# vitasoftAI/ImageRetrievalResearch

Measured on AMD Instinct MI355X. Metric: images/sec embed + queries/sec top-k@100k-gallery, EffNet-B3a 224^2, higher is better.
Workload: dtype bf16

## Files before the change

imageretrievalresearch_amd/csrc/mbconv_block.hip:

```cpp
#include "ops.h"

namespace mi355 {

typedef __bf16 bf16x8 __attribute__((ext_vector_type(8)));
typedef float f32x4 __attribute__((ext_vector_type(4)));
typedef unsigned u32x4 __attribute__((ext_vector_type(4)));
typedef unsigned u32x2 __attribute__((ext_vector_type(2)));

constexpr int MB_THREADS = 512;
constexpr int MB_WAVES = MB_THREADS / 64;
constexpr int MB_MAX_RD = 192;
constexpr int MB_MC = MB_WAVES * 16;

__device__ __forceinline__ float mb_lo(unsigned u) { return __uint_as_float(u << 16); }
__device__ __forceinline__ float mb_hi(unsigned u) { return __uint_as_float(u & 0xffff0000u); }

__device__ __forceinline__ void mb_lds_barrier() {
    asm volatile("s_waitcnt lgkmcnt(0)" ::: "memory");
    __builtin_amdgcn_s_barrier();
    asm volatile("" ::: "memory");
}

__host__ __device__ static inline int mb_proj_ntw(int NTp, int MTp, int NTW) {
    int best = 1, best_busy = 0;
// ... 13 lines not shown
    if (wi != 14) return ntw;
    const int nwn = (NTp + ntw - 1) / ntw;
    int msplit = nwn <= MB_WAVES ? MB_WAVES / nwn : 1;
    if (msplit > MTp) msplit = MTp;
    if (nwn <= MB_WAVES && (MTp + msplit - 1) / msplit <= mwp) return ntw;
    return 4;
}

template <int KS> struct MbTaps {
    static constexpr int KK = KS * KS;
    static constexpr int NV = (KS / 2) * KS;
    static constexpr int NH = (KS + 1) / 2;
    static constexpr int NP = NV + NH;
    __host__ __device__ static constexpr bool vertical(int tp) { return tp < NV; }
    __host__ __device__ static constexpr int tap_a(int tp) {
        return tp < NV ? (tp / KS) * 2 * KS + tp % KS : (KS - 1) * KS + (tp - NV) * 2;
    }
    __host__ __device__ static constexpr int tap_b(int tp) {
        return tp < NV ? tap_a(tp) + KS : ((tp - NV) * 2 + 1 < KS ? tap_a(tp) + 1 : -1);
    }
};

template <int KS, int S, int WI, int MW, int MH, int NTW, int MWP, int KST, int A_IT, int ACT_E, int ACT_D>
__global__ __launch_bounds__(MB_THREADS) void k_mbconv_block(const BlockArgs a) {
    using TP = MbTaps<KS>;
    constexpr int MC = MB_MC;
    constexpr int PAD = KS / 2;
    constexpr int NP = TP::NP;
    constexpr int EW = WI + 2 * PAD;
    constexpr int WO = (WI + 2 * PAD - KS) / S + 1;
    constexpr int TR = WO <= 8 ? 2 : 1;
    constexpr int RP = (TR == 2 && S == 1) ? ((EW + 7) & ~7) : EW;
    static_assert(WO <= 16, "depthwise tile geometry");
    constexpr bool PROJ_WHOLE = WI == 7 && NTW == 2;
    constexpr int KC = WI == 7 ? 256 : 128;
    constexpr int ALD = KC + 16;
    extern __shared__ __attribute__((aligned(16))) unsigned char mb_smem[];

    const int tid = threadIdx.x, lane = tid & 63;
    const int wave = __builtin_amdgcn_readfirstlane(tid >> 6);
    const int fr = lane & 15, fq = lane >> 4, fk = fq * 8;
    const int b = blockIdx.x;
    const int P = a.H * a.W, MT = (P + 15) >> 4, XLD = a.XLD;
    const int EH = a.H + 2 * PAD;
    const int EP = (EH + (TR == 2 ? S : 0)) * RP + 8;
    const int Pout = a.Ho * a.Wo;
    const int MTo = TR == 2 ? (a.Ho + 1) >> 1 : a.Ho;
    const int midp = (a.mid + 15) & ~15;

    bf16_t* Xs = reinterpret_cast<bf16_t*>(mb_smem);
    size_t off = ((size_t)MT * 16 * XLD * 2 + 64 + 15) & ~(size_t)15;
    float* pool = reinterpret_cast<float*>(mb_smem + off);
    off += (size_t)((a.mid + 255) & ~255) * 4;
    float* rvec = reinterpret_cast<float*>(mb_smem + off);
    off += MB_MAX_RD * 4;
    unsigned char* R = mb_smem + off;
    bf16_t* Es = reinterpret_cast<bf16_t*>(R) + (size_t)wave * EP * 16;

    const bool stamping = a.stamps != nullptr;
    unsigned t_acc[8] = {0, 0, 0, 0, 0, 0, 0, 0};
    unsigned t_last = 0;
    if (stamping) t_last = (unsigned)__builtin_readcyclecounter();
    auto tick = [&](int i) {
        if (stamping) { const unsigned t = (unsigned)__builtin_readcyclecounter(); t_acc[i] += t - t_last; t_last = t; }
    };
// ... 10 lines not shown
        for (int h = 0; h < KST; ++h) wq[h] = *reinterpret_cast<const u32x4*>(a.We + (n * a.Kp + fk + h * 32));
        be_reg = *reinterpret_cast<const f32x4*>(a.be + min(cbase + wave * 16 + fq * 4, midp - 4));
        __builtin_amdgcn_sched_barrier(0);
    };
    unsigned short wd_raw[NP], wd_nxt[NP];
    f32x4 bd_reg, bd_nxt;
    auto wd_fetch = [&](int cbase) {
        const int ch = min(cbase + wave * 16 + fr, a.mid - 1);
#pragma unroll
        for (int tp = 0; tp < NP; ++tp) {
            const int ta = TP::tap_a(tp), tb = TP::tap_b(tp) < 0 ? TP::tap_a(tp) : TP::tap_b(tp);
            const int t = (lane & 32) ? tb : ta;
            wd_nxt[tp] = a.Wd[t * a.mid + ch];
        }
        bd_nxt = *reinterpret_cast<const f32x4*>(a.bd + min(cbase + wave * 16 + fq * 4, a.mid - 4));
        __builtin_amdgcn_sched_barrier(0);
    };

    w_prefetch_slab(slab_of(0) * MC);
    wd_fetch(slab_of(0) * MC);
    {
        const int kc = (a.Cin + 7) >> 3;
        const int kcl = XLD >> 3;
        const bf16_t* xb = a.X + (size_t)b * P * a.Cin;
        const int total = MT * 16 * kcl;
        constexpr int U = 9;
        for (int id0 = tid; id0 < total; id0 += MB_THREADS * U) {
            u32x4 v[U];
            int dst[U];
#pragma unroll
            for (int u = 0; u < U; ++u) {
                const int id = id0 + u * MB_THREADS;
                const int row = id / kcl, c = id - row * kcl;
                const u32x4 t = *reinterpret_cast<const u32x4*>(xb + (min(row, P - 1) * a.Cin + min(c, kc - 1) * 8));
                const bool ok = id < total && row < P && c < kc;
                v[u] = ok ? t : (u32x4){0u, 0u, 0u, 0u};
                dst[u] = id < total ? row * XLD + c * 8 : -1;
            }
            if (id0 == tid) {
                bf16_t* Eall = reinterpret_cast<bf16_t*>(R);
                for (int id = tid; id < MB_WAVES * EP * 2; id += MB_THREADS)
                    *reinterpret_cast<u32x4*>(&Eall[id * 8]) = (u32x4){0u, 0u, 0u, 0u};
                if (tid < 4) *reinterpret_cast<u32x4*>(&Xs[MT * 16 * XLD + tid * 8]) = (u32x4){0u, 0u, 0u, 0u};
            }
#pragma unroll
            for (int u = 0; u < U; ++u)
                if (dst[u] >= 0) *reinterpret_cast<u32x4*>(&Xs[dst[u]]) = v[u];
        }
    }
    mb_lds_barrier();
    tick(0);

    bf16_t* Db = a.D + (size_t)b * Pout * a.mid;

    const int e_cv = (fq & 1) * 8 + ((fq >> 1) ? RP * 16 : 0);
    const int e_ch = (fq & 1) * 8 + ((fq >> 1) ? 16 : 0);
    const int t_row = TR == 2 ? (fr >> 3) : 0, t_col = TR == 2 ? (fr & 7) : fr;
    const int e_lane = (t_row * S * RP + t_col * S) * 16;
    constexpr int E_TILE = TR * S * RP * 16;
    const bool col_ok = t_col < WO;

    const int abl = a.variant;
    bool prev_active = false;
    for (int ci = 0; ci < nslabs; ++ci) {
        const int cbase = slab_of(ci) * MC;
        const int ch0 = cbase + wave * 16;
        const bool active = ch0 < a.mid;
        {
            constexpr int MTO_SQ = TR == 2 ? (WO + 1) / 2 : WO;
            if (ci > 0 && prev_active && MTo == MTO_SQ) {
                if constexpr (MTO_SQ >= 14) asm volatile("s_waitcnt vmcnt(14)" ::: "memory");
                else if constexpr (MTO_SQ >= 4) asm volatile("s_waitcnt vmcnt(4)" ::: "memory");
                else asm volatile("s_waitcnt vmcnt(1)" ::: "memory");
            } else {
                asm volatile("s_waitcnt vmcnt(0)" ::: "memory");
            }
// ... 436 lines not shown
                        for (int i = 0; i < MWP; ++i) paf[0][i] = *reinterpret_cast<const bf16x8*>(&as[prow[i] + kk * 32]);
                    }
                    __builtin_amdgcn_sched_barrier(0);
                    if (wactive && ch * KPC + kk < KST2) {
    #pragma unroll
                        for (int i = 0; i < MWP; ++i)
    #pragma unroll
                            for (int j = 0; j < NTW; ++j)
                                acc[j][i] = __builtin_amdgcn_mfma_f32_16x16x32_bf16(*reinterpret_cast<bf16x8*>(&cq[kk][j]), paf[AHEAD ? (kk & 1) : 0][i], acc[j][i], 0, 0, 0);
                    }
                    if ((kk & 1) == 1 && ch + 1 < nchunks) {
                        __builtin_amdgcn_sched_barrier(0);
                        c_fetch(ch + 1, kk - 1);
                        c_fetch(ch + 1, kk);
                        __builtin_amdgcn_sched_barrier(0);
                    }
                }
                tick(6);
                mb_lds_barrier();
                tick(6);
            }
        }
        if (wactive) {
            bf16_t* Yb = a.Y + (size_t)b * Pout * a.Cout;
            const bf16_t* Xb = a.X + (size_t)b * P * a.Cin;
            u32x2 rr[NTW][MWP];
            if (a.has_res) {
#pragma unroll
                for (int i = 0; i < MWP; ++i)
#pragma unroll
                    for (int j = 0; j < NTW; ++j) {
                        const int m = min((mt0 + i) * 16 + fr, Pout - 1);
                        const int n = min((wn * ntw + j) * 16 + fq * 4, a.res_n - 4);
                        rr[j][i] = *reinterpret_cast<const u32x2*>(Xb + (m * a.Cin + n));
                    }
                __builtin_amdgcn_sched_barrier(0);
            }
#pragma unroll
            for (int i = 0; i < MWP; ++i) {
                const int m = (mt0 + i) * 16 + fr;
                if (i < mper && m < Pout) {
#pragma unroll
                    for (int j = 0; j < NTW; ++j) {
                        const int n = (wn * ntw + j) * 16 + fq * 4;
                        if (j < ntw && n < a.Cout) {
                            float v[4] = {acc[j][i].x, acc[j][i].y, acc[j][i].z, acc[j][i].w};
                            if (a.has_res && n < a.res_n) {
                                v[0] += mb_lo(rr[j][i].x); v[1] += mb_hi(rr[j][i].x); v[2] += mb_lo(rr[j][i].y); v[3] += mb_hi(rr[j][i].y);
                            }
                            u32x2 o;
                            o.x = pack2bf(v[0], v[1]);
                            o.y = pack2bf(v[2], v[3]);
                            *reinterpret_cast<u32x2*>(Yb + (m * a.Cout + n)) = o;
                        }
                    }
                }
            }
        }
    }
    tick(7);
    if (stamping && tid == 0) {
        long long* o = a.stamps + (size_t)b * 16;
#pragma unroll
        for (int i = 0; i < 8; ++i) o[i] = (long long)t_acc[i];
    }
}

struct MbGeom { int wi, mw, mh, ntw, mwp, a_it; };
static bool mb_geom(int H, int W, MbGeom* g) {
    if (W == 7 && H * W <= 64) { *g = {7, 4, 1, 3, 4, 4}; return true; }
    if (W == 14 && H * W <= 208) { *g = {14, 7, 2, 3, 7, 7}; return true; }
    return false;
}
#define MB_INSTANCES(X)                                                                                              \
    X(3, 1, 14, 3, 3, ACT_SILU) X(5, 1, 14, 3, 3, ACT_SILU) X(5, 1, 14, 5, 3, ACT_SILU) X(5, 2, 14, 5, 2, ACT_SILU)     \
    X(5, 1, 7, 8, 2, ACT_SILU) X(3, 1, 7, 8, 3, ACT_SILU) X(3, 1, 7, 12, 3, ACT_SILU)                                 \
    X(3, 1, 14, 4, 2, ACT_NONE) X(3, 1, 14, 4, 3, ACT_NONE) X(3, 1, 14, 5, 3, ACT_NONE) X(3, 1, 14, 6, 3, ACT_NONE)   \
    X(3, 1, 7, 7, 2, ACT_NONE) X(3, 1, 7, 8, 2, ACT_NONE) X(3, 1, 7, 8, 3, ACT_NONE) X(3, 1, 7, 9, 3, ACT_NONE)       \
    X(3, 1, 7, 10, 3, ACT_NONE) X(3, 1, 7, 11, 3, ACT_NONE) X(3, 1, 14, 6, 4, ACT_NONE)
static bool mb_instance_ok(int k, int stride, int wi, int kst, int ntw, int act_d) {
#define X(KS, S, WI, KST, NTW, AD) if (k == KS && stride == S && wi == WI && kst == KST && ntw == NTW && act_d == AD) return true;
    MB_INSTANCES(X)
#undef X
    return false;
}

static int mb_pick_kcs(const BlockArgs& a) {
    const int Pout = a.Ho * a.Wo;
    const int q = a.W == 7 ? 256 : 128;
    const size_t pl = (size_t)((a.mid + 255) & ~255) * 4;
    const long avail = 160l * 1024 - (long)pl;
    const int kmax = (int)((avail / Pout / 2 - 16) / q) * q;
    if (kmax < q) return 0;
    const int nsc = (a.Kp2 + kmax - 1) / kmax;
    const int per = (a.Kp2 + nsc - 1) / nsc;
    return (per + q - 1) / q * q;
}

static size_t mb_lds_bytes_xld(const BlockArgs& a, int k, int xld, const MbGeom& g) {
    const int P = a.H * a.W, MT = (P + 15) / 16, pad = k / 2;
    const int wo = a.Wo, ew = a.W + 2 * pad;
    const int stride = (a.H + 2 * pad - k) / (a.Ho > 1 ? a.Ho - 1 : 1) >= 2 ? 2 : 1;
    const int rp = (wo <= 8 && stride == 1) ? ((ew + 7) & ~7) : ew;
    const int EP = (a.H + 2 * pad + (wo <= 8 ? stride : 0)) * rp + 8;
    const size_t xs = ((size_t)MT * 16 * xld * 2 + 64 + 15) & ~(size_t)15, pl = (size_t)((a.mid + 255) & ~255) * 4;
    const size_t fixed = xs + pl + MB_MAX_RD * 4;
    const size_t slab = (size_t)MB_WAVES * EP * 16 * 2;
// ... 28 lines not shown
    if (act_e != ACT_SILU) return false;
    if (Cin % 8 || mid % 8 || mid > 2560 || Cout % 8 || rd < 1 || rd > MB_MAX_RD) return false;
    if (!((k == 3 || k == 5) && (stride == 1 || stride == 2))) return false;
    if (W == 7 && stride == 2) return false;
    if ((long)mid * ((Cin + 31) & ~31) >= (1l << 30) || (long)Cout * mid >= (1l << 30)) return false;
    BlockArgs a{};
    a.H = H; a.W = W; a.Cin = Cin; a.Kp = (Cin + 31) & ~31; a.mid = mid; a.Cout = Cout;
    const int pad = k / 2;
    a.Ho = (H + 2 * pad - k) / stride + 1; a.Wo = (W + 2 * pad - k) / stride + 1;
    const int Pout = a.Ho * a.Wo, MTp = (Pout + 15) / 16, NTp = (Cout + 15) / 16;
    const int ntw = mb_pick_ntw(NTp, MTp, g.wi, g.mwp);
    const int nwn = (NTp + ntw - 1) / ntw;
    if (nwn > MB_WAVES) return false;
    int msplit = MB_WAVES / nwn;
    if (msplit > MTp) msplit = MTp;
    if ((MTp + msplit - 1) / msplit > g.mwp) return false;
    a.Kp2 = (mid + 31) & ~31;
    if (Pout * (g.wi == 7 ? 32 : 16) > g.a_it * MB_THREADS) return false;
    if ((H * W + 15) / 16 > g.mw * g.mh) return false;
    if (!mb_instance_ok(k, stride, g.wi, a.Kp / 32, ntw, act_d)) return false;
    return mb_pick_xld(a, k, g) != 0;
}

template <int KS, int S, int WI, int MW, int MH, int NTW, int MWP, int KST, int A_IT, int ACT_E, int ACT_D>
static int launch_mb(BlockArgs a, int B, hipStream_t st) {
    MbGeom g;
    mb_geom(a.H, a.W, &g);
    a.XLD = mb_pick_xld(a, KS, g);
    a.KCS = mb_pick_kcs(a);
    const size_t lds = mb_lds_bytes_xld(a, KS, a.XLD, g);
    static bool attr_done[64] = {false};
    int dev = 0;
    MI355_CHECK_HIP(hipGetDevice(&dev));
    if (dev >= 0 && dev < 64 && !attr_done[dev]) {
        MI355_CHECK_HIP(hipFuncSetAttribute((const void*)k_mbconv_block<KS, S, WI, MW, MH, NTW, MWP, KST, A_IT, ACT_E, ACT_D>,
                                            hipFuncAttributeMaxDynamicSharedMemorySize, 160 * 1024));
        attr_done[dev] = true;
    }
    hipLaunchKernelGGL((k_mbconv_block<KS, S, WI, MW, MH, NTW, MWP, KST, A_IT, ACT_E, ACT_D>), dim3(B), dim3(MB_THREADS), lds, st, a);
    MI355_LAUNCH_CHECK();
    return OK;
}

int launch_mbconv_block(const BlockArgs& a, int B, int k, int stride, hipStream_t st) {
    MI355_REQUIRE(mbconv_block_supported(a.H, a.W, a.Cin, a.mid, a.Cout, k, stride, a.rd, a.act_e, a.act_d), "mbconv_block: unsupported shape");
    const int Pout = a.Ho * a.Wo;
    MbGeom gg;
    mb_geom(a.H, a.W, &gg);
    const int ntw = mb_pick_ntw((a.Cout + 15) / 16, (Pout + 15) / 16, gg.wi, gg.mwp);
    const int kst = a.Kp / 32;
#define X(KS, S, WI, KST, NTW, AD)                                                                  \
    if (k == KS && stride == S && a.W == WI && kst == KST && ntw == NTW && a.act_d == AD)           \
        return launch_mb<KS, S, WI, (WI == 7 ? 4 : 7), (WI == 7 ? 1 : 2), NTW, (WI == 7 ? 4 : 7), KST, (WI == 7 ? 4 : 7), ACT_SILU, AD>(a, B, st);
    MB_INSTANCES(X)
#undef X
    set_error("mbconv_block: no instance for k=%d s=%d W=%d Kp=%d ntw=%d", k, stride, a.W, a.Kp, ntw);
    return ERR_UNSUPPORTED;
}

}
```

imageretrievalresearch_amd/csrc/model.hip:

```cpp
#include "model_exec.h"
#include "../../include/mi355_retrieval.h"

#include <string.h>

#include <algorithm>

namespace mi355 {

int pack_gemm(Packer& pk, Op& op) {
    const TensorSpec* w = pk.get(op.w_name);
    if (!w) return ERR_STATE;
    const int N = op.cout_real, K = op.cin_real;
    MI355_REQUIRE(w->numel() == (int64_t)N * K, "pack: %s has %lld elements, expected %d x %d", op.w_name.c_str(),
                  (long long)w->numel(), N, K);
    std::vector<float> scale, shift;
    if (!pk.bn_fold(op.bn_name, op.bn_eps, N, scale, shift)) return ERR_STATE;
    if (!op.bias_name.empty()) {
        const TensorSpec* b = pk.get(op.bias_name);
        if (!b) return ERR_STATE;
        for (int i = 0; i < N; ++i) shift[i] = b->data[i] * scale[i] + shift[i];
    }
    const int Np = (op.cout + 15) & ~15, Kp = (op.cin + 31) & ~31;
    op.w_off = pk.alloc((size_t)Np * Kp * 2);
    op.b_off = pk.alloc((size_t)Np * 4);
// ... 318 lines not shown
    if (g.out != SLOT_E || d.in != SLOT_E || d.out != SLOT_D || p.in != SLOT_D || !p.use_gate || !d.pool) return false;
    if (g.use_gate || g.res != SLOT_NONE || g.a_relu6 || !g.tap.empty() || !d.tap.empty()) return false;
    if (p.act != ACT_NONE || (p.res != SLOT_NONE && p.res != g.in)) return false;
    if (p.res != SLOT_NONE && p.res_channels && ((p.res_channels + 7) & ~7) != g.cin) return false;
    return mbconv_block_supported(h, w, g.cin, g.cout, p.cout, d.k, d.stride, s.rd, g.act, d.act);
}

static int stamp_ptr(ExecCtx& cx, size_t oi, long long** out) {
    mi355_model* m = cx.m;
    *out = nullptr;
    if (!m->block_stamps) return OK;
    const size_t need = m->def.ops.size() * (size_t)cx.B * 16 * sizeof(long long);
    if (m->stamp_bytes < need) {
        if (m->stamp_buf) MI355_CHECK_HIP(hipFree(m->stamp_buf));
        MI355_CHECK_HIP(hipMalloc((void**)&m->stamp_buf, need));
        m->stamp_bytes = need;
    }
    m->stamp_B = cx.B;
    *out = m->stamp_buf + (oi * (size_t)cx.B + cx.b0) * 16;
    MI355_CHECK_HIP(hipMemsetAsync(*out, 0, (size_t)cx.nb * 16 * sizeof(long long), cx.st));
    return OK;
}

static int exec_block(ExecCtx& cx, size_t oi) {
    mi355_model* m = cx.m;
    SlotState* S = m->slots;
    const Op& g = m->def.ops[oi];
    const Op& d = m->def.ops[oi + 1];
    const Op& s = m->def.ops[oi + 2];
    const Op& p = m->def.ops[oi + 3];
    BlockArgs a{};
    a.X = (const bf16_t*)cx.slot_ptr(g.in);
    a.We = (const bf16_t*)cx.w(g.w_off); a.be = (const float*)cx.w(g.b_off);
    a.Wd = (const bf16_t*)cx.w(d.w_off); a.bd = (const float*)cx.w(d.b_off);
    a.W1 = (const bf16_t*)cx.w(s.w3_off); a.b1 = (const float*)cx.w(s.b_off);
    a.W2 = (const bf16_t*)cx.w(s.w4_off); a.b2 = (const float*)cx.w(s.b2_off);
    a.Wp = (const bf16_t*)cx.w(p.w_off); a.bp = (const float*)cx.w(p.b_off);
    a.D = (bf16_t*)cx.slot_ptr(d.out);
    a.Y = (bf16_t*)cx.slot_ptr(p.out);
    a.H = S[g.in].h; a.W = S[g.in].w; a.Cin = g.cin; a.Kp = (g.cin + 31) & ~31; a.mid = g.cout;
    a.Ho = S[d.out].h; a.Wo = S[d.out].w; a.Cout = p.cout; a.Kp2 = (p.cin + 31) & ~31; a.rd = s.rd;
    a.has_res = p.res != SLOT_NONE;
    a.res_n = p.res != SLOT_NONE ? (p.res_channels ? ((p.res_channels + 7) & ~7) : p.cout) : 0;
    a.a_relu6 = p.a_relu6;
    a.act_e = g.act; a.act_d = d.act; a.se_act = s.se_act;
    a.inv_hw = 1.0f / (float)(a.Ho * a.Wo);
    a.norot = m->block_norot;
    a.variant = m->block_variant;
    a.stamps = nullptr;
    { const int rc = stamp_ptr(cx, oi, &a.stamps); if (rc != OK) return rc; }
    return launch_mbconv_block(a, cx.nb, d.k, d.stride, cx.st);
}

static int exec_fused(ExecCtx& cx, const Op& g, const Op& d) {
    mi355_model* m = cx.m;
    SlotState* S = m->slots;
    FusedArgs a{};
    a.X = (const bf16_t*)cx.slot_ptr(g.in);
    a.We = (const bf16_t*)cx.w(g.w_off); a.be = (const float*)cx.w(g.b_off);
    a.Wd = (const bf16_t*)cx.w(d.w_off); a.bd = (const float*)cx.w(d.b_off);
    a.D = (bf16_t*)cx.slot_ptr(d.out);
    a.pool = d.pool ? (float*)cx.slot_ptr(SLOT_POOLPART) : nullptr;
    a.H = S[g.in].h; a.W = S[g.in].w; a.Cin = g.cin; a.Kp = (g.cin + 31) & ~31; a.mid = g.cout;
    a.Ho = S[d.out].h; a.Wo = S[d.out].w; a.act_e = g.act; a.act_d = d.act;
    a.debug_skip = m->fuse_debug;
    if (fused_late_supported(a.H, a.W, g.cin, g.cout, d.k, d.stride)) {
        m->pool_nblk = 1;
        return launch_fused_late(a, cx.nb, d.k, d.stride, cx.st);
    }
    if (use_sweep(m, g, d, a.H, a.W)) {
        SweepArgs sa{};
        sa.X = a.X; sa.We = a.We; sa.be = a.be; sa.Wd = a.Wd; sa.bd = a.bd; sa.D = a.D; sa.pool = a.pool;
        sa.H = a.H; sa.W = a.W; sa.Cin = a.Cin; sa.Kp = a.Kp; sa.mid = a.mid; sa.Ho = a.Ho; sa.Wo = a.Wo;
        sa.act_e = a.act_e; sa.act_d = a.act_d; sa.csplit_override = m->sweep_csplit; sa.variant = m->sweep_variant; sa.debug_skip = m->sweep_skip;
// ... 6 lines not shown
    return launch_fused_band(a, cx.nb, d.k, d.stride, cx.st);
}

static void op_range_label(const Op& op, int H, int W, int in_h, int in_w, const char* how, char* lab, size_t n) {
    switch (op.kind) {
        case OP_STEM: snprintf(lab, n, "embed/%sstem 3->%d @%dx%d", how, op.cout_real, conv_out(H, 3, 2), conv_out(W, 3, 2)); break;
        case OP_GEMM: snprintf(lab, n, "embed/%spw %d->%d @%dx%d%s%s", how, op.cin_real, op.cout_real, in_h, in_w,
                               op.use_gate ? " gate" : "", op.res != SLOT_NONE ? " res" : ""); break;
        case OP_DW: snprintf(lab, n, "embed/%sdw k%d s%d C%d @%dx%d", how, op.k, op.stride, op.cin_real, in_h, in_w); break;
        case OP_SE: snprintf(lab, n, "embed/%sse C%d rd%d", how, op.cin_real, op.rd); break;
        default: snprintf(lab, n, "embed/%sop%d C%d->%d t%d", how, (int)op.kind, op.cin_real, op.cout_real, op.tokens_h); break;
    }
}

static int run_backbone(ExecCtx& cx, size_t op_begin = 0, size_t op_end = (size_t)-1) {
    mi355_model* m = cx.m;
    SlotState* S = m->slots;
    if (op_end > m->def.ops.size()) op_end = m->def.ops.size();
    for (size_t oi = op_begin; oi < op_end; ++oi) {
        const Op& op = m->def.ops[oi];
        const int op_index = (int)oi;
        const int in_h = S[op.in == SLOT_NONE ? 0 : op.in].h, in_w = S[op.in == SLOT_NONE ? 0 : op.in].w;
        const bool block = op.in != SLOT_NONE && can_fuse_block(m, oi, in_h, in_w, cx.B);
        const bool fused = block || can_fuse(m, oi, in_h, in_w);
        if (fused) {
            const Op& d = m->def.ops[oi + 1];
            S[op.out].h = S[op.in].h; S[op.out].w = S[op.in].w; S[op.out].c = op.cout;
            S[d.out].h = conv_out(S[op.in].h, d.k, d.stride); S[d.out].w = conv_out(S[op.in].w, d.k, d.stride);
            S[d.out].c = d.cout;
            if (block) {
                const Op& pj = m->def.ops[oi + 3];
                S[pj.out].h = S[d.out].h; S[pj.out].w = S[d.out].w; S[pj.out].c = pj.cout;
            }
        } else
        switch (op.kind) {
            case OP_STEM: S[op.out].h = conv_out(cx.H, 3, 2); S[op.out].w = conv_out(cx.W, 3, 2); S[op.out].c = op.cout; break;
            case OP_GEMM: S[op.out].h = S[op.in].h; S[op.out].w = S[op.in].w; S[op.out].c = op.cout; break;
            case OP_DW: {
                const int ho = conv_out(S[op.in].h, op.k, op.stride), wo = conv_out(S[op.in].w, op.k, op.stride);
                S[op.out].h = ho; S[op.out].w = wo; S[op.out].c = op.cout;
                break;
            }
            case OP_SE: break;
            default: if (op.out != SLOT_NONE) { S[op.out].h = op.tokens_h; S[op.out].w = op.tokens_h; S[op.out].c = op.cout; } break;
        }
        hipEvent_t e0 = nullptr, e1 = nullptr;
// ... 167 lines not shown
    m->def.num_classes = num_classes;
    const std::string n = name;
    int e;
    if (n == "efficientnet_b3a" || n == "efficientnet_b3") e = build_efficientnet_b3(m->def);
    else if (n == "rexnet_100") e = build_rexnet(m->def, 1.0);
    else if (n == "rexnet_130") e = build_rexnet(m->def, 1.3);
    else if (n == "rexnet_150") e = build_rexnet(m->def, 1.5);
    else if (n == "rexnet_200") e = build_rexnet(m->def, 2.0);
    else if (n == "swin_base_patch4_window7_224") e = build_swin_base(m->def);
    else {
        set_error("Unknown model name '%s'. Known: efficientnet_b3a, rexnet_100/130/150/200, swin_base_patch4_window7_224", name);
        e = ERR_ARG;
    }
    if (e) { delete m; return e; }
    *out = m;
    return OK;
}

void mi355_model_destroy(mi355_model_t m) {
    if (!m) return;
    if (m->dev_blob) (void)hipFree(m->dev_blob);
    if (m->arena) (void)hipFree(m->arena);
    if (m->stamp_buf) (void)hipFree(m->stamp_buf);
    for (int l = 0; l < 4; ++l) {
        if (m->lane_stream[l]) (void)hipStreamDestroy(m->lane_stream[l]);
        if (m->lane_join[l]) (void)hipEventDestroy(m->lane_join[l]);
    }
    if (m->lane_fork) (void)hipEventDestroy(m->lane_fork);
    for (auto& kv : m->tapbufs)
        if (kv.second.ptr) (void)hipFree(kv.second.ptr);
    delete m;
}

int mi355_model_num_tensors(mi355_model_t m) { return m ? (int)m->def.tensors.size() : 0; }

int mi355_model_tensor_info(mi355_model_t m, int i, const char** name, int* ndim, int64_t shape[4], int* kind) {
    MI355_REQUIRE(m && i >= 0 && i < (int)m->def.tensors.size(), "tensor_info: index %d out of range", i);
    const TensorSpec& t = m->def.tensors[i];
    if (name) *name = t.name.c_str();
    if (ndim) *ndim = (int)t.shape.size();
    if (shape)
        for (int d = 0; d < 4; ++d) shape[d] = d < (int)t.shape.size() ? t.shape[d] : 1;
    if (kind) *kind = t.kind;
    return OK;
}

// ... 61 lines not shown
    size_t i0 = ops.size(), i1 = ops.size();
    for (size_t i = 0; i < ops.size(); ++i) {
        if (ops[i].tap == from_tap) i0 = i;
        if (ops[i].tap == to_tap) i1 = i;
    }
    MI355_REQUIRE(i0 < ops.size() && i1 < ops.size() && i0 < i1, "run_between_taps: taps '%s' -> '%s' not found in that order",
                  from_tap, to_tap);
    const Op& src = ops[i0];
    MI355_REQUIRE(src.out != SLOT_NONE && (src.cout_real ? src.cout_real : src.cout) == C,
                  "run_between_taps: tap '%s' has %d channels, got %d", from_tap, src.cout_real ? src.cout_real : src.cout, C);
    hipStream_t st = (hipStream_t)stream;
    int H = 32, W = 32;
    for (const Op& op : ops) { (void)op; }
    {
        int sh = 1;
        for (size_t i = 0; i <= i0; ++i)
            if (ops[i].kind == OP_STEM || (ops[i].kind == OP_DW && ops[i].stride == 2)) sh *= 2;
        H = h * sh; W = w * sh;
    }
    const size_t bytes = plan_slots(m, B, H, W);
    m->lane_bytes = 0;
    if (int e = ensure_arena(m, bytes)) return e;
    ExecCtx cx{m, st, B, H, W, nullptr, 0, B};
    SlotState* S = m->slots;
    S[src.out].h = h; S[src.out].w = w; S[src.out].c = src.cout;
    if (int e = launch_nchw_f32_to_nhwc_bf16(x, (bf16_t*)cx.slot_ptr(src.out), B, h * w, C, src.cout, st)) return e;
    return run_backbone(cx, i0 + 1, i1 + 1);
}

int mi355_model_forward_u8(mi355_model_t m, const unsigned char* images, int B, int h, int w, int fill, const float* mean,
                           const float* stdv, const float* conv_input_w, int features_only, float* out, float* pooled_out,
                           void* stream) {
    MI355_REQUIRE(m && images && mean && stdv && out, "forward_u8: null pointer");
    MI355_REQUIRE(B >= 1 && h >= 1 && w >= 1 && h <= 16384 && w <= 16384, "forward_u8: bad image size %dx%d", h, w);
    MI355_REQUIRE(fill >= 0 && fill <= 255, "forward_u8: fill must be a byte value");
    for (int c = 0; c < 3; ++c) MI355_REQUIRE(stdv[c] != 0.f, "forward_u8: std[%d] is zero", c);
    MI355_REQUIRE(!m->def.ops.empty() && (m->def.ops[0].kind == OP_STEM || m->def.ops[0].kind == OP_PATCH_EMBED),
                  "forward_u8: %s has no stem / patch embedding to fuse the pre-processing into", m->def.arch.c_str());
    MI355_REQUIRE(m->def.ops[0].kind == OP_STEM || !conv_input_w, "forward_u8: conv_input belongs to the convolutional backbones");
    U8Source u{};
    u.img = images; u.h = h; u.w = w; u.fill = fill; u.conv_w = conv_input_w;
    for (int c = 0; c < 3; ++c) { u.mean[c] = mean[c]; u.stdv[c] = stdv[c]; }
    const int S = h > w ? h : w;
    return forward_impl(m, nullptr, B, S, S, out, pooled_out, features_only != 0, (hipStream_t)stream, &u);
}

// ... 61 lines not shown
    MI355_REQUIRE(it != m->tapbufs.end(), "read_tap: no tap named '%s' was recorded", tap_name);
    const TapBuf& t = it->second;
    if (shape) { shape[0] = t.B; shape[1] = t.c_real; shape[2] = t.h; shape[3] = t.w; }
    if (!out) return OK;
    MI355_REQUIRE(out_numel >= (int64_t)t.B * t.c_real * t.h * t.w, "read_tap: output too small");
    return launch_nhwc_to_nchw_f32((const bf16_t*)t.ptr, out, t.B, t.h * t.w, t.c, t.c_real, (hipStream_t)stream);
}

int mi355_model_set_option(mi355_model_t m, const char* key, int64_t value) {
    MI355_REQUIRE(m && key, "set_option: null argument");
    const std::string k = key;
    if (k == "microbatch") m->microbatch = (int)value;
    else if (k == "lanes") m->lanes = (int)value;
    else if (k == "fuse") m->fuse = value != 0;
    else if (k == "fuse_band") m->fuse_band = (int)value;
    else if (k == "fuse_sweep") m->fuse_sweep = (int)value;
    else if (k == "sweep_csplit") m->sweep_csplit = (int)value;
    else if (k == "sweep_variant") m->sweep_variant = (int)value;
    else if (k == "sweep_skip") m->sweep_skip = (int)value;
    else if (k == "fuse_debug") m->fuse_debug = (int)value;
    else if (k == "fuse_ln") m->fuse_ln = (int)value;
    else if (k == "fuse_block") m->fuse_block = (int)value;
    else if (k == "fuse_block_min_batch") m->fuse_block_min_batch = (int)value;
    else if (k == "block_stamps") m->block_stamps = value != 0;
    else if (k == "block_norot") m->block_norot = (int)value;
    else if (k == "block_variant") m->block_variant = (int)value;
    else if (k == "fuse_head_gap") m->fuse_head_gap = value != 0;
    else if (k == "roctx") roctx_enable(value != 0);
    else if (k == "profile") {
        m->profile = value != 0;
        for (int i = 0; i < PK_COUNT; ++i) { m->prof_ms[i] = 0; m->prof_launches[i] = 0; }
        m->prof_op_ms.assign(m->def.ops.size(), 0.0);
        m->prof_op_n.assign(m->def.ops.size(), 0);
    } else {
        set_error("set_option: unknown option '%s'", key);
        return ERR_ARG;
    }
    return OK;
}

int mi355_model_profile_read(mi355_model_t m, double* ms_by_kind, int64_t* launches_by_kind, int n) {
    MI355_REQUIRE(m && ms_by_kind && launches_by_kind && n >= PK_COUNT, "profile_read: need arrays of >= %d", PK_COUNT);
    for (auto& pe : m->prof_events) {
        MI355_CHECK_HIP(hipEventSynchronize(pe.second.second));
        float ms = 0.f;
        MI355_CHECK_HIP(hipEventElapsedTime(&ms, pe.second.first, pe.second.second));
// ... 233 lines not shown
```

imageretrievalresearch_amd/csrc/model_exec.h:

```cpp
#pragma once
#include "model.h"

#include <string.h>

namespace mi355 {

int swin_exec(const ModelDef& def, const Op& op, struct ExecCtx& cx);

static inline uint16_t f2bf_host(float f) {
    uint32_t u;
    memcpy(&u, &f, 4);
    if ((u & 0x7fffffffu) > 0x7f800000u) return (uint16_t)((u >> 16) | 0x40);
    u += 0x7fffu + ((u >> 16) & 1u);
    return (uint16_t)(u >> 16);
}
static inline float bf_round_host(float f) {
    uint32_t u = ((uint32_t)f2bf_host(f)) << 16;
    float r;
    memcpy(&r, &u, 4);
    return r;
}

struct SlotState {
    size_t off = 0, bytes = 0;
// ... 15 lines not shown
struct mi355_model {
    ModelDef def;
    std::vector<char> blob;
    void* dev_blob = nullptr;
    size_t dev_blob_bytes = 0;
    bool packed = false;
    void* arena = nullptr;
    size_t arena_bytes = 0;
    int arena_device = -1, blob_device = -1;
    SlotState slots[SLOT_COUNT];
    int microbatch = 0;
    int lanes = 1;
    hipStream_t lane_stream[4] = {nullptr, nullptr, nullptr, nullptr};
    hipEvent_t lane_fork = nullptr, lane_join[4] = {nullptr, nullptr, nullptr, nullptr};
    size_t lane_bytes = 0;
    int fuse_sweep = 1;
    int sweep_variant = 0, sweep_skip = 0;
    int sweep_csplit = 0;
    int fuse_band = 2;
    bool fuse = true;
    int fuse_block = 1;
    int fuse_block_min_batch = 96;
    bool fuse_head_gap = true;
    int block_variant = 0;
    int block_norot = 0;
    bool block_stamps = false;
    long long* stamp_buf = nullptr; size_t stamp_bytes = 0; int stamp_B = 0;
    int fuse_debug = 0;
    int fuse_ln = 1;
    int pool_nblk = 0;
    bool taps = false;
    std::map<std::string, TapBuf> tapbufs;
    bool profile = false;
    std::vector<std::pair<int, std::pair<hipEvent_t, hipEvent_t>>> prof_events;
    std::vector<char> prof_fused;
    std::vector<double> prof_op_ms;
    std::vector<long> prof_op_n;
    double prof_ms[PK_COUNT] = {0};
    long prof_launches[PK_COUNT] = {0};
};

namespace mi355 {

struct ExecCtx {
    mi355_model* m;
    hipStream_t st;
    int nb, H, W;
    const float* x;
    int b0, B;
    int lane = 0;
    const unsigned char* x_u8 = nullptr;
    int img_h = 0, img_w = 0, fill = 255;
    float mean[3] = {0.f, 0.f, 0.f}, stdv[3] = {1.f, 1.f, 1.f};
    const float* conv_w = nullptr;
    const int64_t* u8_desc = nullptr;
    int ln_pending_in = SLOT_NONE;
    char* base() const { return (char*)m->arena + (size_t)lane * m->lane_bytes; }
    void* slot_ptr(int s) const { return s == SLOT_NONE ? nullptr : base() + m->slots[s].off; }
    const char* w(size_t off) const { return (const char*)m->dev_blob + off; }
};

struct Packer {
    mi355_model* m;
    std::vector<char>& blob;
    size_t alloc(size_t bytes) {
        const size_t off = align_up(blob.size(), 256);
        blob.resize(off + bytes, 0);
        return off;
    }
    const TensorSpec* get(const std::string& name) {
        auto it = m->def.index.find(name);
        if (it == m->def.index.end()) { set_error("pack: unknown tensor '%s'", name.c_str()); return nullptr; }
        const TensorSpec& t = m->def.tensors[it->second];
        if (!t.set) { set_error("pack: tensor '%s' was never set (mi355_model_set_tensor)", name.c_str()); return nullptr; }
        return &t;
    }
    bool bn_fold(const std::string& bn, float eps, int n, std::vector<float>& scale, std::vector<float>& shift) {
        scale.assign(n, 1.f);
        shift.assign(n, 0.f);
// ... 17 lines not shown
```

imageretrievalresearch_amd/csrc/ops.h:

```cpp
#pragma once
#include "common.h"

namespace mi355 {

struct GemmArgs {
    const bf16_t* A; int lda;
    const bf16_t* W; int ldw;
    const float* bias;
    const bf16_t* res; int ldr; int res_n;
    const float* gate; int gate_ld; int rows_per_img;
    void* out; int ldo; int out_f32;
    int M, N, K;
    int act;
    int a_relu6;
    const bf16_t* zeros;
    long M_sel;
    float* splitk_ws;
    size_t splitk_ws_bytes;
    const float* ln_stats;
    const float* ln_colsum;
};
int launch_gemm_bf16(const GemmArgs& a, hipStream_t st, int* path = nullptr);
bool gemm_wide_supported(const GemmArgs& a);
int launch_gemm_wide(const GemmArgs& a, hipStream_t st);
// ... 37 lines not shown
bool sweep_mbconv_supported(int H, int W, int Cin, int mid, int k, int stride, int act_e, int act_d);
int launch_sweep_mbconv(const SweepArgs& a, int B, int k, int stride, hipStream_t st);

struct BlockArgs {
    const bf16_t* X;
    const bf16_t* We; const float* be;
    const bf16_t* Wd; const float* bd;
    const bf16_t* W1; const float* b1;
    const bf16_t* W2; const float* b2;
    const bf16_t* Wp; const float* bp;
    bf16_t* D;
    bf16_t* Y;
    long long* stamps;
    int H, W, Cin, Kp, mid, Ho, Wo, Cout, Kp2, rd;
    int XLD;
    int KCS;
    int norot;
    int variant;
    int has_res;
    int res_n;
    int a_relu6;
    int act_e, act_d, se_act;
    float inv_hw;
};
bool mbconv_block_supported(int H, int W, int Cin, int mid, int Cout, int k, int stride, int rd, int act_e, int act_d);
int launch_mbconv_block(const BlockArgs& a, int B, int k, int stride, hipStream_t st);

int launch_stem(const float* x, const float* w, const float* bias, bf16_t* out, int B, int H, int W, int Cout,
                int act, hipStream_t st);

int launch_stem_u8(const unsigned char* img, int h, int w, int fill, const float* mean, const float* stdv,
                   const float* conv_w, const float* sw, const float* bias, bf16_t* out, int B, int Cout, int act,
                   hipStream_t st, const int64_t* desc = nullptr, int b0 = 0);

int check_images(const unsigned char* pixels, int64_t pixels_bytes, const int64_t* desc_host, const int64_t* desc_dev, int B,
                 const char* who);
size_t resize_batch_workspace(const int64_t* desc_host, int B, int out_h, int out_w, bool pad);
int resize_batch(const unsigned char* pixels, int64_t pixels_bytes, const int64_t* desc_host, const int64_t* desc_dev, int B,
                 int out_h, int out_w, bool pad, int fill, unsigned char* out, void* workspace, size_t workspace_bytes,
                 hipStream_t st);

int dw_pool_blocks(int Ho, int Wo, int C);
int launch_dwconv(const bf16_t* in, const bf16_t* w, const float* bias, bf16_t* out, float* pool_partial, int B,
                  int H, int W, int C, int k, int stride, int act, int* pool_nblk, hipStream_t st);

int launch_se(const float* pool_partial, int nblk, float inv_hw, const float* w1, const float* b1, const float* w2,
              const float* b2, float* gate, int B, int C, int rd, int act1, hipStream_t st);

int launch_gap(const bf16_t* in, float* pooled, bf16_t* pooled_bf16, int B, int HW, int C, hipStream_t st);
// ... 17 lines not shown
```

Measured before the change: 60270.

## Fuse consecutive MBConv blocks into one persistent chain kernel launch

Adds a chain kernel that runs several consecutive fused MBConv blocks inside one launch. Each workgroup handles one image and dispatches per-block template instances through a switch over a device-side entry table. Intermediate outputs ping-pong between two halves of the E slot, with per-entry batch strides. The aim is to remove per-block launch overhead and inter-kernel gaps and to keep each image's data hot in cache. The cost is a much larger combined kernel, which risks register pressure and code bloat and makes occupancy follow the worst block. It also adds host-side table management with an async memcpy when entries change.

New measurement: 60230 (median of 6 runs). Within noise of the previous version (-0.1%).

```diff
diff --git a/imageretrievalresearch_amd/csrc/mbconv_block.hip b/imageretrievalresearch_amd/csrc/mbconv_block.hip
--- a/imageretrievalresearch_amd/csrc/mbconv_block.hip
+++ b/imageretrievalresearch_amd/csrc/mbconv_block.hip
@@ -59,7 +59,7 @@
 };
 
 template <int KS, int S, int WI, int MW, int MH, int NTW, int MWP, int KST, int A_IT, int ACT_E, int ACT_D>
-__global__ __launch_bounds__(MB_THREADS) void k_mbconv_block(const BlockArgs a) {
+__device__ __forceinline__ void mb_block_body(const BlockArgs& a, const int b, const int tid) {
     using TP = MbTaps<KS>;
     constexpr int MC = MB_MC;
     constexpr int PAD = KS / 2;
@@ -74,10 +74,9 @@
     constexpr int ALD = KC + 16;
     extern __shared__ __attribute__((aligned(16))) unsigned char mb_smem[];
 
-    const int tid = threadIdx.x, lane = tid & 63;
+    const int lane = tid & 63;
     const int wave = __builtin_amdgcn_readfirstlane(tid >> 6);
     const int fr = lane & 15, fq = lane >> 4, fk = fq * 8;
-    const int b = blockIdx.x;
     const int P = a.H * a.W, MT = (P + 15) >> 4, XLD = a.XLD;
     const int EH = a.H + 2 * PAD;
     const int EP = (EH + (TR == 2 ? S : 0)) * RP + 8;
@@ -134,7 +133,7 @@
     {
         const int kc = (a.Cin + 7) >> 3;
         const int kcl = XLD >> 3;
-        const bf16_t* xb = a.X + (size_t)b * P * a.Cin;
+        const bf16_t* xb = a.X + (size_t)b * a.xs;
         const int total = MT * 16 * kcl;
         constexpr int U = 9;
         for (int id0 = tid; id0 < total; id0 += MB_THREADS * U) {
@@ -163,7 +162,7 @@
     mb_lds_barrier();
     tick(0);
 
-    bf16_t* Db = a.D + (size_t)b * Pout * a.mid;
+    bf16_t* Db = a.D + (size_t)b * a.ds;
 
     const int e_cv = (fq & 1) * 8 + ((fq >> 1) ? RP * 16 : 0);
     const int e_ch = (fq & 1) * 8 + ((fq >> 1) ? 16 : 0);
@@ -646,8 +645,8 @@
             }
         }
         if (wactive) {
-            bf16_t* Yb = a.Y + (size_t)b * Pout * a.Cout;
-            const bf16_t* Xb = a.X + (size_t)b * P * a.Cin;
+            bf16_t* Yb = a.Y + (size_t)b * a.ys;
+            const bf16_t* Xb = a.X + (size_t)b * a.xs;
             u32x2 rr[NTW][MWP];
             if (a.has_res) {
 #pragma unroll
@@ -690,6 +689,11 @@
     }
 }
 
+template <int KS, int S, int WI, int MW, int MH, int NTW, int MWP, int KST, int A_IT, int ACT_E, int ACT_D>
+__global__ __launch_bounds__(MB_THREADS) void k_mbconv_block(const BlockArgs a) {
+    mb_block_body<KS, S, WI, MW, MH, NTW, MWP, KST, A_IT, ACT_E, ACT_D>(a, blockIdx.x, threadIdx.x);
+}
+
 struct MbGeom { int wi, mw, mh, ntw, mwp, a_it; };
 static bool mb_geom(int H, int W, MbGeom* g) {
     if (W == 7 && H * W <= 64) { *g = {7, 4, 1, 3, 4, 4}; return true; }
@@ -702,11 +706,48 @@
     X(3, 1, 14, 4, 2, ACT_NONE) X(3, 1, 14, 4, 3, ACT_NONE) X(3, 1, 14, 5, 3, ACT_NONE) X(3, 1, 14, 6, 3, ACT_NONE)   \
     X(3, 1, 7, 7, 2, ACT_NONE) X(3, 1, 7, 8, 2, ACT_NONE) X(3, 1, 7, 8, 3, ACT_NONE) X(3, 1, 7, 9, 3, ACT_NONE)       \
     X(3, 1, 7, 10, 3, ACT_NONE) X(3, 1, 7, 11, 3, ACT_NONE) X(3, 1, 14, 6, 4, ACT_NONE)
+#define MB_TARGS(KS, S, WI, KST, NTW, AD) \
+    KS, S, WI, (WI == 7 ? 4 : 7), (WI == 7 ? 1 : 2), NTW, (WI == 7 ? 4 : 7), KST, (WI == 7 ? 4 : 7), ACT_SILU, AD
+struct MbInst { int ks, s, wi, kst, ntw, ad; };
+#define X(KS, S, WI, KST, NTW, AD) MbInst{KS, S, WI, KST, NTW, AD},
+constexpr MbInst MB_TABLE[] = {MB_INSTANCES(X)};
+#undef X
+constexpr int MB_NINST = sizeof(MB_TABLE) / sizeof(MB_TABLE[0]);
+__host__ __device__ constexpr int mb_inst_id(int k, int stride, int wi, int kst, int ntw, int act_d) {
+    for (int i = 0; i < MB_NINST; ++i) {
+        const MbInst& t = MB_TABLE[i];
+        if (t.ks == k && t.s == stride && t.wi == wi && t.kst == kst && t.ntw == ntw && t.ad == act_d) return i;
+    }
+    return -1;
+}
 static bool mb_instance_ok(int k, int stride, int wi, int kst, int ntw, int act_d) {
-#define X(KS, S, WI, KST, NTW, AD) if (k == KS && stride == S && wi == WI && kst == KST && ntw == NTW && act_d == AD) return true;
-    MB_INSTANCES(X)
+    return mb_inst_id(k, stride, wi, kst, ntw, act_d) >= 0;
+}
+
+template <int ACT_D>
+__global__ __launch_bounds__(MB_THREADS) void k_mbconv_chain(const MbChainEntry* ents, int n) {
+#if defined(__HIP_DEVICE_COMPILE__)
+    typedef const __attribute__((address_space(4))) MbChainEntry* CPtr;
+#else
+    typedef const MbChainEntry* CPtr;
+#endif
+    const CPtr ce = (CPtr)ents;
+    for (int i = 0; i < n; ++i) {
+        if (i > 0) __syncthreads();
+        int b = blockIdx.x, tid = threadIdx.x;
+        asm volatile("" : "+s"(b));
+        asm volatile("" : "+v"(tid));
+        const BlockArgs a = ce[i].a;
+        switch (ce[i].inst) {
+#define X(KS, S, WI, KST, NTW, AD) \
+            case mb_inst_id(KS, S, WI, KST, NTW, AD):                                                                 \
+                if constexpr (AD == ACT_D) mb_block_body<MB_TARGS(KS, S, WI, KST, NTW, AD)>(a, b, tid);                 \
+                break;
+            MB_INSTANCES(X)
 #undef X
-    return false;
+            default: break;
+        }
+    }
 }
 
 static int mb_pick_kcs(const BlockArgs& a) {
@@ -781,40 +822,73 @@
     return mb_pick_xld(a, k, g) != 0;
 }
 
-template <int KS, int S, int WI, int MW, int MH, int NTW, int MWP, int KST, int A_IT, int ACT_E, int ACT_D>
-static int launch_mb(BlockArgs a, int B, hipStream_t st) {
+static int mb_prepare(BlockArgs& a, int k, int stride, size_t* lds) {
     MbGeom g;
     mb_geom(a.H, a.W, &g);
-    a.XLD = mb_pick_xld(a, KS, g);
+    a.XLD = mb_pick_xld(a, k, g);
     a.KCS = mb_pick_kcs(a);
-    const size_t lds = mb_lds_bytes_xld(a, KS, a.XLD, g);
-    static bool attr_done[64] = {false};
+    if (!a.xs) a.xs = a.H * a.W * a.Cin;
+    if (!a.ds) a.ds = a.Ho * a.Wo * a.mid;
+    if (!a.ys) a.ys = a.Ho * a.Wo * a.Cout;
+    *lds = mb_lds_bytes_xld(a, k, a.XLD, g);
+    const int Pout = a.Ho * a.Wo;
+    const int ntw = mb_pick_ntw((a.Cout + 15) / 16, (Pout + 15) / 16, g.wi, g.mwp);
+    return mb_inst_id(k, stride, g.wi, a.Kp / 32, ntw, a.act_d);
+}
+
+static int mb_lds_attr(const void* fn, bool (&done)[64]) {
     int dev = 0;
     MI355_CHECK_HIP(hipGetDevice(&dev));
-    if (dev >= 0 && dev < 64 && !attr_done[dev]) {
-        MI355_CHECK_HIP(hipFuncSetAttribute((const void*)k_mbconv_block<KS, S, WI, MW, MH, NTW, MWP, KST, A_IT, ACT_E, ACT_D>,
-                                            hipFuncAttributeMaxDynamicSharedMemorySize, 160 * 1024));
-        attr_done[dev] = true;
-    }
+    if (dev >= 0 && dev < 64 && !done[dev]) {
+        MI355_CHECK_HIP(hipFuncSetAttribute(fn, hipFuncAttributeMaxDynamicSharedMemorySize, 160 * 1024));
+        done[dev] = true;
+    }
+    return OK;
+}
+
+template <int KS, int S, int WI, int MW, int MH, int NTW, int MWP, int KST, int A_IT, int ACT_E, int ACT_D>
+static int launch_mb(const BlockArgs& a, size_t lds, int B, hipStream_t st) {
+    static bool attr_done[64] = {false};
+    if (int e = mb_lds_attr((const void*)k_mbconv_block<KS, S, WI, MW, MH, NTW, MWP, KST, A_IT, ACT_E, ACT_D>, attr_done)) return e;
     hipLaunchKernelGGL((k_mbconv_block<KS, S, WI, MW, MH, NTW, MWP, KST, A_IT, ACT_E, ACT_D>), dim3(B), dim3(MB_THREADS), lds, st, a);
     MI355_LAUNCH_CHECK();
     return OK;
 }
 
-int launch_mbconv_block(const BlockArgs& a, int B, int k, int stride, hipStream_t st) {
-    MI355_REQUIRE(mbconv_block_supported(a.H, a.W, a.Cin, a.mid, a.Cout, k, stride, a.rd, a.act_e, a.act_d), "mbconv_block: unsupported shape");
-    const int Pout = a.Ho * a.Wo;
-    MbGeom gg;
-    mb_geom(a.H, a.W, &gg);
-    const int ntw = mb_pick_ntw((a.Cout + 15) / 16, (Pout + 15) / 16, gg.wi, gg.mwp);
-    const int kst = a.Kp / 32;
-#define X(KS, S, WI, KST, NTW, AD)                                                                  \
-    if (k == KS && stride == S && a.W == WI && kst == KST && ntw == NTW && a.act_d == AD)           \
-        return launch_mb<KS, S, WI, (WI == 7 ? 4 : 7), (WI == 7 ? 1 : 2), NTW, (WI == 7 ? 4 : 7), KST, (WI == 7 ? 4 : 7), ACT_SILU, AD>(a, B, st);
+int launch_mbconv_block(const BlockArgs& a0, int B, int k, int stride, hipStream_t st) {
+    MI355_REQUIRE(mbconv_block_supported(a0.H, a0.W, a0.Cin, a0.mid, a0.Cout, k, stride, a0.rd, a0.act_e, a0.act_d), "mbconv_block: unsupported shape");
+    BlockArgs a = a0;
+    size_t lds = 0;
+    const int id = mb_prepare(a, k, stride, &lds);
+#define X(KS, S, WI, KST, NTW, AD) \
+    if (id == mb_inst_id(KS, S, WI, KST, NTW, AD)) return launch_mb<MB_TARGS(KS, S, WI, KST, NTW, AD)>(a, lds, B, st);
     MB_INSTANCES(X)
 #undef X
-    set_error("mbconv_block: no instance for k=%d s=%d W=%d Kp=%d ntw=%d", k, stride, a.W, a.Kp, ntw);
+    set_error("mbconv_block: no instance for k=%d s=%d W=%d Kp=%d", k, stride, a.W, a.Kp);
     return ERR_UNSUPPORTED;
 }
 
-}
+size_t mbconv_chain_entry(const BlockArgs& a, int k, int stride, MbChainEntry* e) {
+    *e = MbChainEntry{};
+    if (!mbconv_block_supported(a.H, a.W, a.Cin, a.mid, a.Cout, k, stride, a.rd, a.act_e, a.act_d)) return 0;
+    e->a = a;
+    size_t lds = 0;
+    e->inst = mb_prepare(e->a, k, stride, &lds);
+    return e->inst >= 0 ? lds : 0;
+}
+
+int mbconv_chain_family(const MbChainEntry& e) { return e.inst >= 0 && e.inst < MB_NINST ? MB_TABLE[e.inst].ad : -1; }
+
+bool mbconv_chain_family_supported(int family) { return family == ACT_SILU; }
+
+int launch_mbconv_chain(const MbChainEntry* entries, int n, int family, size_t lds, int B, hipStream_t st) {
+    MI355_REQUIRE(entries && n >= 1 && B >= 1 && lds >= 1 && lds <= 160 * 1024, "mbconv_chain: bad arguments");
+    MI355_REQUIRE(mbconv_chain_family_supported(family), "mbconv_chain: no chain kernel for family %d", family);
+    static bool attr_done[64] = {false};
+    if (int e = mb_lds_attr((const void*)k_mbconv_chain<ACT_SILU>, attr_done)) return e;
+    hipLaunchKernelGGL(k_mbconv_chain<ACT_SILU>, dim3(B), dim3(MB_THREADS), lds, st, entries, n);
+    MI355_LAUNCH_CHECK();
+    return OK;
+}
+
+}
diff --git a/imageretrievalresearch_amd/csrc/model.hip b/imageretrievalresearch_amd/csrc/model.hip
--- a/imageretrievalresearch_amd/csrc/model.hip
+++ b/imageretrievalresearch_amd/csrc/model.hip
@@ -364,9 +364,8 @@
     return OK;
 }
 
-static int exec_block(ExecCtx& cx, size_t oi) {
+static BlockArgs block_args(ExecCtx& cx, size_t oi, int h, int w, int ho, int wo) {
     mi355_model* m = cx.m;
-    SlotState* S = m->slots;
     const Op& g = m->def.ops[oi];
     const Op& d = m->def.ops[oi + 1];
     const Op& s = m->def.ops[oi + 2];
@@ -380,8 +379,8 @@
     a.Wp = (const bf16_t*)cx.w(p.w_off); a.bp = (const float*)cx.w(p.b_off);
     a.D = (bf16_t*)cx.slot_ptr(d.out);
     a.Y = (bf16_t*)cx.slot_ptr(p.out);
-    a.H = S[g.in].h; a.W = S[g.in].w; a.Cin = g.cin; a.Kp = (g.cin + 31) & ~31; a.mid = g.cout;
-    a.Ho = S[d.out].h; a.Wo = S[d.out].w; a.Cout = p.cout; a.Kp2 = (p.cin + 31) & ~31; a.rd = s.rd;
+    a.H = h; a.W = w; a.Cin = g.cin; a.Kp = (g.cin + 31) & ~31; a.mid = g.cout;
+    a.Ho = ho; a.Wo = wo; a.Cout = p.cout; a.Kp2 = (p.cin + 31) & ~31; a.rd = s.rd;
     a.has_res = p.res != SLOT_NONE;
     a.res_n = p.res != SLOT_NONE ? (p.res_channels ? ((p.res_channels + 7) & ~7) : p.cout) : 0;
     a.a_relu6 = p.a_relu6;
@@ -390,8 +389,121 @@
     a.norot = m->block_norot;
     a.variant = m->block_variant;
     a.stamps = nullptr;
+    return a;
+}
+
+static int exec_block(ExecCtx& cx, size_t oi) {
+    SlotState* S = cx.m->slots;
+    const Op& g = cx.m->def.ops[oi];
+    const Op& d = cx.m->def.ops[oi + 1];
+    BlockArgs a = block_args(cx, oi, S[g.in].h, S[g.in].w, S[d.out].h, S[d.out].w);
     { const int rc = stamp_ptr(cx, oi, &a.stamps); if (rc != OK) return rc; }
     return launch_mbconv_block(a, cx.nb, d.k, d.stride, cx.st);
+}
+
+static bool read_before_write(const mi355_model* m, size_t from, int slot) {
+    for (size_t i = from; i < m->def.ops.size(); ++i) {
+        const Op& op = m->def.ops[i];
+        if (op.in == slot || op.res == slot || (op.use_gate && slot == SLOT_GATE)) return true;
+        if (op.out == slot) return false;
+    }
+    return false;
+}
+
+static int exec_chain(ExecCtx& cx, size_t oi, size_t op_end, int* launched) {
+    mi355_model* m = cx.m;
+    SlotState* S = m->slots;
+    const auto& ops = m->def.ops;
+    *launched = 0;
+    if (!m->fuse_chain || m->profile || m->block_stamps || m->taps || !cx.chain_ok) return OK;
+    struct Blk { size_t oi; int h, w, ho, wo; };
+    std::vector<Blk> run;
+    {
+        int h = S[ops[oi].in].h, w = S[ops[oi].in].w;
+        for (size_t j = oi; j + 3 < op_end && ops[j].in != SLOT_NONE && can_fuse_block(m, j, h, w, cx.B); j += 4) {
+            if (!run.empty() && ops[j].in != ops[run.back().oi + 3].out) break;
+            const Op& d = ops[j + 1];
+            const Blk bk{j, h, w, conv_out(h, d.k, d.stride), conv_out(w, d.k, d.stride)};
+            run.push_back(bk);
+            h = bk.ho; w = bk.wo;
+        }
+    }
+    std::vector<MbChainEntry> ents;
+    for (size_t n = run.size(); n >= 2; --n) {
+        const Blk& f = run[0];
+        const Blk& l = run[n - 1];
+        const Op& g0 = ops[f.oi];
+        const Op& pl = ops[l.oi + 3];
+        const int s_in = g0.in, s_out = pl.out;
+        if (s_in == SLOT_E || s_in == SLOT_D || s_out == SLOT_E || s_out == SLOT_D) continue;
+        const long x0 = (long)f.h * f.w * g0.cin, yl = (long)l.ho * l.wo * pl.cout;
+        if (s_in == s_out && x0 != yl) continue;
+        long ymax = 0, dmax = 0;
+        for (size_t k = 0; k < n; ++k) {
+            const Blk& bk = run[k];
+            if (k + 1 < n) ymax = std::max(ymax, (long)bk.ho * bk.wo * ops[bk.oi + 3].cout);
+            dmax = std::max(dmax, (long)bk.ho * bk.wo * ops[bk.oi].cout);
+        }
+        const size_t half = (S[SLOT_E].bytes / 2) & ~(size_t)255;
+        if ((size_t)cx.nb * ymax * 2 > half || (size_t)cx.nb * dmax * 2 > S[SLOT_D].bytes) continue;
+        const size_t after = l.oi + 4;
+        bool stale = read_before_write(m, after, SLOT_E) || read_before_write(m, after, SLOT_D);
+        for (size_t k = 0; k + 1 < n && !stale; ++k) {
+            const int so = ops[run[k].oi + 3].out;
+            if (so != s_out && read_before_write(m, after, so)) stale = true;
+        }
+        if (stale) continue;
+        bf16_t* ebuf[2] = {(bf16_t*)cx.slot_ptr(SLOT_E), (bf16_t*)((char*)cx.slot_ptr(SLOT_E) + half)};
+        ents.assign(n, MbChainEntry{});
+        size_t lds = 0;
+        int family = -1;
+        bool ok = true;
+        for (size_t k = 0; k < n && ok; ++k) {
+            const Blk& bk = run[k];
+            BlockArgs a = block_args(cx, bk.oi, bk.h, bk.w, bk.ho, bk.wo);
+            if (k > 0) { a.X = ebuf[(k - 1) & 1]; a.xs = (int)ymax; }
+            if (k + 1 < n) { a.Y = ebuf[k & 1]; a.ys = (int)ymax; }
+            a.ds = (int)dmax;
+            const Op& d = ops[bk.oi + 1];
+            const size_t l_k = mbconv_chain_entry(a, d.k, d.stride, &ents[k]);
+            const int fam = mbconv_chain_family(ents[k]);
+            ok = l_k > 0 && mbconv_chain_family_supported(fam) && (family < 0 || fam == family);
+            family = fam;
+            lds = std::max(lds, l_k);
+        }
+        if (!ok) continue;
+        const size_t nops = ops.size(), base = (size_t)cx.lane * nops + f.oi;
+        int dev = 0;
+        MI355_CHECK_HIP(hipGetDevice(&dev));
+        if (!m->chain_dev || m->chain_device != dev || m->chain_host.size() != 4 * nops) {
+            if (m->chain_dev) (void)hipFree(m->chain_dev);
+            m->chain_dev = nullptr;
+            MI355_CHECK_HIP(hipMalloc((void**)&m->chain_dev, 4 * nops * sizeof(MbChainEntry)));
+            m->chain_device = dev;
+            m->chain_host.assign(4 * nops, MbChainEntry{});
+            for (auto& e : m->chain_host) e.inst = -1;
+        }
+        if (memcmp(&m->chain_host[base], ents.data(), n * sizeof(MbChainEntry)) != 0) {
+            memcpy(&m->chain_host[base], ents.data(), n * sizeof(MbChainEntry));
+            MI355_CHECK_HIP(hipMemcpyAsync(m->chain_dev + base, &m->chain_host[base], n * sizeof(MbChainEntry), hipMemcpyHostToDevice, cx.st));
+        }
+        char lab[96] = "";
+        if (roctx_active()) snprintf(lab, sizeof lab, "embed/block chain: %d blocks from op %d", (int)n, (int)f.oi);
+        RoctxRange range(lab);
+        if (int e = launch_mbconv_chain(m->chain_dev + base, (int)n, family, lds, cx.nb, cx.st)) return e;
+        for (size_t k = 0; k < n; ++k) {
+            const Blk& bk = run[k];
+            const Op& g = ops[bk.oi];
+            const Op& d = ops[bk.oi + 1];
+            const Op& p = ops[bk.oi + 3];
+            S[g.out].h = bk.h; S[g.out].w = bk.w; S[g.out].c = g.cout;
+            S[d.out].h = bk.ho; S[d.out].w = bk.wo; S[d.out].c = d.cout;
+            S[p.out].h = bk.ho; S[p.out].w = bk.wo; S[p.out].c = p.cout;
+        }
+        *launched = (int)n;
+        return OK;
+    }
+    return OK;
 }
 
 static int exec_fused(ExecCtx& cx, const Op& g, const Op& d) {
@@ -444,6 +556,11 @@
         const int op_index = (int)oi;
         const int in_h = S[op.in == SLOT_NONE ? 0 : op.in].h, in_w = S[op.in == SLOT_NONE ? 0 : op.in].w;
         const bool block = op.in != SLOT_NONE && can_fuse_block(m, oi, in_h, in_w, cx.B);
+        if (block) {
+            int n = 0;
+            if (int e = exec_chain(cx, oi, op_end, &n)) return e;
+            if (n > 0) { oi += 4 * (size_t)n - 1; continue; }
+        }
         const bool fused = block || can_fuse(m, oi, in_h, in_w);
         if (fused) {
             const Op& d = m->def.ops[oi + 1];
@@ -657,6 +774,7 @@
     if (m->dev_blob) (void)hipFree(m->dev_blob);
     if (m->arena) (void)hipFree(m->arena);
     if (m->stamp_buf) (void)hipFree(m->stamp_buf);
+    if (m->chain_dev) (void)hipFree(m->chain_dev);
     for (int l = 0; l < 4; ++l) {
         if (m->lane_stream[l]) (void)hipStreamDestroy(m->lane_stream[l]);
         if (m->lane_join[l]) (void)hipEventDestroy(m->lane_join[l]);
@@ -764,6 +882,7 @@
     m->lane_bytes = 0;
     if (int e = ensure_arena(m, bytes)) return e;
     ExecCtx cx{m, st, B, H, W, nullptr, 0, B};
+    cx.chain_ok = false;
     SlotState* S = m->slots;
     S[src.out].h = h; S[src.out].w = w; S[src.out].c = src.cout;
     if (int e = launch_nchw_f32_to_nhwc_bf16(x, (bf16_t*)cx.slot_ptr(src.out), B, h * w, C, src.cout, st)) return e;
@@ -871,6 +990,7 @@
     else if (k == "fuse_ln") m->fuse_ln = (int)value;
     else if (k == "fuse_block") m->fuse_block = (int)value;
     else if (k == "fuse_block_min_batch") m->fuse_block_min_batch = (int)value;
+    else if (k == "fuse_chain") m->fuse_chain = (int)value;
     else if (k == "block_stamps") m->block_stamps = value != 0;
     else if (k == "block_norot") m->block_norot = (int)value;
     else if (k == "block_variant") m->block_variant = (int)value;
diff --git a/imageretrievalresearch_amd/csrc/model_exec.h b/imageretrievalresearch_amd/csrc/model_exec.h
--- a/imageretrievalresearch_amd/csrc/model_exec.h
+++ b/imageretrievalresearch_amd/csrc/model_exec.h
@@ -61,6 +61,10 @@
     int fuse_block = 1;
     int fuse_block_min_batch = 96;
     bool fuse_head_gap = true;
+    int fuse_chain = 1;
+    MbChainEntry* chain_dev = nullptr;
+    int chain_device = -1;
+    std::vector<MbChainEntry> chain_host;
     int block_variant = 0;
     int block_norot = 0;
     bool block_stamps = false;
@@ -94,6 +98,7 @@
     const float* conv_w = nullptr;
     const int64_t* u8_desc = nullptr;
     int ln_pending_in = SLOT_NONE;
+    bool chain_ok = true;
     char* base() const { return (char*)m->arena + (size_t)lane * m->lane_bytes; }
     void* slot_ptr(int s) const { return s == SLOT_NONE ? nullptr : base() + m->slots[s].off; }
     const char* w(size_t off) const { return (const char*)m->dev_blob + off; }
diff --git a/imageretrievalresearch_amd/csrc/ops.h b/imageretrievalresearch_amd/csrc/ops.h
--- a/imageretrievalresearch_amd/csrc/ops.h
+++ b/imageretrievalresearch_amd/csrc/ops.h
@@ -83,9 +83,19 @@
     int a_relu6;
     int act_e, act_d, se_act;
     float inv_hw;
+    int xs, ds, ys;
 };
 bool mbconv_block_supported(int H, int W, int Cin, int mid, int Cout, int k, int stride, int rd, int act_e, int act_d);
 int launch_mbconv_block(const BlockArgs& a, int B, int k, int stride, hipStream_t st);
+struct MbChainEntry {
+    BlockArgs a;
+    int inst;
+    int pad_[3];
+};
+size_t mbconv_chain_entry(const BlockArgs& a, int k, int stride, MbChainEntry* e);
+int mbconv_chain_family(const MbChainEntry& e);
+bool mbconv_chain_family_supported(int family);
+int launch_mbconv_chain(const MbChainEntry* entries, int n, int family, size_t lds, int B, hipStream_t st);
 
 int launch_stem(const float* x, const float* w, const float* bias, bf16_t* out, int B, int H, int W, int Cout,
                 int act, hipStream_t st);
```
